# russellgeum/Digging-into-Self-Supervised-Monocular-Depth-Estimation

Measured on AMD Instinct MI355X. Metric: images/sec training, KITTI 192x640 batch 12/GPU, higher is better.
Workload: dtype f32; 1 GPU; configs[1]: kitti_eigen_zhou-shaped 192x640, batch 12/GPU, ResNet18 depth + separate ResNet18 pose, frame_ids [0,-1,1], 4 scales, automask, Adam, fp32; global_batch=12, parallelism=dp1

## Files before the change

### digging-into-self-supervised-monocular-depth-estimation_amd/csrc/norm_nhwc.hip

```cpp
#include "nhwc_common.hpp"

namespace mdx {
namespace nhwc {

constexpr int STATS_FWD_BLOCKS = 256;
constexpr int STATS_BWD_BLOCKS_F32 = 256, STATS_BWD_BLOCKS_BF16 = 384;
constexpr int STATS_MAX_BLOCKS = 384;
constexpr int APPLY_MAX_BLOCKS = 4096;
constexpr int STATS_ITERS = 8, APPLY_ITERS = 4;
static inline int stats_bwd_blocks(int dtype) { return dtype == MDX_F32 ? STATS_BWD_BLOCKS_F32 : STATS_BWD_BLOCKS_BF16; }

template <typename T>
__global__ __launch_bounds__(NB) void bn_nhwc_fwd_stats_kernel(const T *__restrict__ x, int M, int C, int CVB, int PL, int RB,
                                                               float *__restrict__ part)
{
    constexpr int N = VecN<T>::N;
    __shared__ float lds[2 * NB * N];
    const Pos p = position<N>(M, C, CVB, PL, RB);
    float a[N], q[N];
#pragma unroll
    for (int j = 0; j < N; ++j) a[j] = q[j] = 0.f;
    if (p.active) {
        const T *px = x + (size_t)p.g * M * C + (size_t)p.cv * N;
        auto acc = [&](const Vec<T, N> &v) {
// ... 241 lines not shown
    auto apply = [&](const Vec<T, N> &vd, const Vec<T, N> &vd2, const Vec<T, N> &vy, const Vec<T, N> &vx, size_t off) {
        Vec<T, N> wx, wr;
#pragma unroll
        for (int j = 0; j < N; ++j) {
            float d = to_float(vd.v[j]);
            if (pd2) d += to_float(vd2.v[j]);
            const float yv = !MASKX ? to_float(vy.v[j]) : to_float(from_float<T>(__builtin_fmaf(to_float(vx.v[j]), k0[j], shift[j])));
            const float dz = (relu && !(yv > 0.f)) ? 0.f : d;
            const float xh = (to_float(vx.v[j]) - mean[j]) * invstd[j];
            wx.v[j] = from_float<T>(k0[j] * (dz - mdz[j] - xh * mdzx[j]));
            wr.v[j] = from_float<T>(dz);
        }
        store_vec<T, N>(ox + off, wx);
        if (orr) store_vec<T, N>(orr + off, wr);
    };
    int r = p.r0 + p.pl;
    for (; r + PL < p.r1; r += 2 * PL) {
        const size_t o0 = (size_t)r * C, o1 = (size_t)(r + PL) * C;
        const Vec<T, N> d0 = load_vec<T, N>(pd + o0), d1 = load_vec<T, N>(pd + o1);
        Vec<T, N> y0 = {}, y1 = {};
        if (!MASKX) { y0 = load_vec<T, N>(py + o0); y1 = load_vec<T, N>(py + o1); }
        const Vec<T, N> x0 = load_vec<T, N>(px + o0), x1 = load_vec<T, N>(px + o1);
        Vec<T, N> e0 = {}, e1 = {};
        if (pd2) { e0 = load_vec<T, N>(pd2 + o0); e1 = load_vec<T, N>(pd2 + o1); }
        apply(d0, e0, y0, x0, o0);
        apply(d1, e1, y1, x1, o1);
    }
    for (; r < p.r1; r += PL) {
        const size_t o = (size_t)r * C;
        Vec<T, N> e = {}, yv = {};
        if (pd2) e = load_vec<T, N>(pd2 + o);
        if (!MASKX) yv = load_vec<T, N>(py + o);
        apply(load_vec<T, N>(pd + o), e, yv, load_vec<T, N>(px + o), o);
    }
}

}
}

using namespace mdx;
using namespace mdx::nhwc;

MDX_EXPORT size_t mdx_bn_nhwc_workspace_bytes(int B, int C, int H, int W, int groups, int dtype)
{
    if (B <= 0 || C <= 0 || H <= 0 || W <= 0 || groups <= 0 || !dtype_ok(dtype)) return 0;
    const Rows g = make_rows((long long)B * H * W, C, vec_elems(dtype), STATS_MAX_BLOCKS, STATS_ITERS);
    return ((size_t)groups * g.nblk * 2 * C + (size_t)groups * 2 * C) * sizeof(float);
}

static int nhwc_args_ok(int B, int C, int H, int W, int groups, int dtype)
{
    if (groups <= 0 || groups > 65535) return MDX_ERR_BAD_SHAPE;
    return nhwc_map_ok(B, C, H, W, dtype);
}

MDX_EXPORT int mdx_bn_act_nhwc_fwd(const void *x, const void *res, const float *gamma, const float *beta, float *run_mean,
                                   float *run_var, void *y, float *save_mean, float *save_invstd, int B, int C, int H, int W,
                                   int groups, float eps, float momentum, int relu, int dtype, void *workspace,
                                   size_t workspace_bytes, void *stream)
{
    if (!x || !gamma || !beta || !y || !save_mean || !save_invstd || !workspace) return MDX_ERR_NULL_POINTER;
    if ((run_mean == nullptr) != (run_var == nullptr)) return MDX_ERR_NULL_POINTER;
    const int bad = nhwc_args_ok(B, C, H, W, groups, dtype);
    if (bad) return bad;
    if (!aligned(x, 16) || !aligned(y, 16) || (res && !aligned(res, 16))) return MDX_ERR_MISALIGNED;
    if (workspace_bytes < mdx_bn_nhwc_workspace_bytes(B, C, H, W, groups, dtype)) return MDX_ERR_WORKSPACE;
    const int M = B * H * W, N = vec_elems(dtype);
    const Rows gs = make_rows(M, C, N, STATS_FWD_BLOCKS, STATS_ITERS), ga = make_rows(M, C, N, APPLY_MAX_BLOCKS, APPLY_ITERS);
    float *part = (float *)workspace;
    hipStream_t st = (hipStream_t)stream;
    const dim3 grid_s(gs.nblk, gs.t.ny, groups), grid_a(ga.nblk, ga.t.ny, groups), block(NB);
    dispatch_dtype(dtype, [&](auto t) {
        using T = typename decltype(t)::type;
        hipLaunchKernelGGL((bn_nhwc_fwd_stats_kernel<T>), grid_s, block, 0, st, (const T *)x, M, C, gs.t.CVB, gs.t.PL, gs.RB, part);
    });
    hipLaunchKernelGGL(bn_nhwc_fwd_finalize_kernel, dim3((C + FC - 1) / FC), dim3(FC * FS), 0, st, part, gs.nblk, C, groups, (double)M,
                       eps, momentum, save_mean, save_invstd, run_mean, run_var);
    dispatch_dtype(dtype, [&](auto t) {
        using T = typename decltype(t)::type;
        hipLaunchKernelGGL((bn_nhwc_fwd_apply_kernel<T>), grid_a, block, 0, st, (const T *)x, (const T *)res, gamma, beta, save_mean,
                           save_invstd, M, C, ga.t.CVB, ga.t.PL, ga.RB, relu, (T *)y);
    });
    return check_launch();
}

MDX_EXPORT int mdx_bn_act_nhwc_bwd(const void *dy, const void *dy2, const void *y, const void *x, const float *gamma,
                                   const float *beta, const float *save_mean, const float *save_invstd, void *dx, void *dres, float *dgamma,
                                   float *dbeta, int B, int C, int H, int W, int groups, int relu, int dtype, void *workspace,
                                   size_t workspace_bytes, void *stream)
{
    if (!dy || !x || !gamma || !save_mean || !save_invstd || !dx || !dgamma || !dbeta || !workspace)
        return MDX_ERR_NULL_POINTER;
    if (!y && (!relu || !beta || dres)) return MDX_ERR_NULL_POINTER;
    const int bad = nhwc_args_ok(B, C, H, W, groups, dtype);
    if (bad) return bad;
    if (!aligned(dy, 16) || (y && !aligned(y, 16)) || !aligned(x, 16) || !aligned(dx, 16) || (dy2 && !aligned(dy2, 16)) ||
        (dres && !aligned(dres, 16)))
        return MDX_ERR_MISALIGNED;
    if (workspace_bytes < mdx_bn_nhwc_workspace_bytes(B, C, H, W, groups, dtype)) return MDX_ERR_WORKSPACE;
    const int M = B * H * W, N = vec_elems(dtype);
    const Rows gs = make_rows(M, C, N, stats_bwd_blocks(dtype), STATS_ITERS), ga = make_rows(M, C, N, APPLY_MAX_BLOCKS, APPLY_ITERS);
    float *part = (float *)workspace;
    float *totals = part + (size_t)groups * gs.nblk * 2 * C;
    hipStream_t st = (hipStream_t)stream;
    const dim3 grid_s(gs.nblk, gs.t.ny, groups), grid_a(ga.nblk, ga.t.ny, groups), block(NB);
    const bool maskx = !y;
    dispatch_dtype_flag(dtype, maskx, [&](auto t, auto mx) {
        using T = typename decltype(t)::type;
        hipLaunchKernelGGL((bn_nhwc_bwd_stats_kernel<T, decltype(mx)::value>), grid_s, block, 0, st, (const T *)dy, (const T *)dy2,
                           (const T *)y, (const T *)x, gamma, beta, save_mean, save_invstd, M, C, gs.t.CVB, gs.t.PL, gs.RB, relu, part);
    });
    hipLaunchKernelGGL(bn_nhwc_bwd_finalize_kernel, dim3((C + FC - 1) / FC), dim3(FC * FS), 0, st, part, gs.nblk, C, groups, (double)M, totals,
                       dgamma, dbeta);
    dispatch_dtype_flag(dtype, maskx, [&](auto t, auto mx) {
        using T = typename decltype(t)::type;
        hipLaunchKernelGGL((bn_nhwc_bwd_apply_kernel<T, decltype(mx)::value>), grid_a, block, 0, st, (const T *)dy, (const T *)dy2,
                           (const T *)y, (const T *)x, gamma, beta, save_mean, save_invstd, totals, M, C, ga.t.CVB, ga.t.PL, ga.RB, relu,
                           (T *)dx, (T *)dres);
    });
    return check_launch();
}
```

### digging-into-self-supervised-monocular-depth-estimation_amd/mdx/functional.py

```python
import ctypes as C

import torch

from . import _lib
from ._lib import api, ptr, stream, workspace


def _f32c(t, keep_format=False):
    if t is not None and t.dtype != torch.float32:
        t = t.float()
    if t is None or t.is_contiguous() or (keep_format and t.is_contiguous(memory_format=torch.channels_last)):
        return t
    return t.contiguous()


def _byref(struct):
    return C.byref(struct) if struct is not None else None


class _ComposeProjection(torch.autograd.Function):
    @staticmethod
    def forward(ctx, K, T):
        K, T = _f32c(K), _f32c(T)
        B = K.shape[0]
        P = torch.empty(B, 3, 4, device=K.device, dtype=torch.float32)
        api.mdx_compose_projection(ptr(K), ptr(T), B, ptr(P), stream())
        ctx.save_for_backward(K, T)
        return P

    @staticmethod
    def backward(ctx, gP):
        K, T = ctx.saved_tensors
        gK = gT = None
# ... 918 lines not shown
        nws = api.mdx_bn_nhwc_workspace_bytes(Bg, Cc, H, W, groups, code) if cl else api.mdx_bn_workspace_bytes(Bg, Cc, H, W)
        ws = workspace(nws, x.device)
        fn = api.mdx_bn_act_nhwc_fwd if cl else api.mdx_bn_act_fwd
        fn(ptr(x, x.dtype, cl=cl), ptr(res, x.dtype, optional=True, cl=cl), ptr(weight), ptr(bias),
           ptr(running_mean, optional=True), ptr(running_var, optional=True), ptr(y, x.dtype, cl=cl), ptr(save_mean),
           ptr(save_invstd), Bg, Cc, H, W, groups, eps, momentum, int(relu), code, ptr(ws, torch.uint8), nws, stream())
        mask_from_x = cl and bool(relu) and res is None and x.dtype == torch.float32
        ctx.save_for_backward(x, bias if mask_from_x else y, weight, save_mean, save_invstd)
        ctx.meta = (bool(relu), res is not None, groups, cl, mask_from_x)
        ctx.mark_non_differentiable(*[t for t in (running_mean, running_var) if t is not None])
        ctx.set_materialize_grads(False)
        return (y, y.view_as(y)) if fork else y

    @staticmethod
    def backward(ctx, dy, dy2=None):
        x, y, weight, save_mean, save_invstd = ctx.saved_tensors
        relu, has_res, groups, cl, mask_from_x = ctx.meta
        bias = None
        if mask_from_x:
            y, bias = None, y
        dy, dy2 = _two_grads(dy, dy2, x.dtype, cl, fused_add=cl)
        if dy is None:
            return (None,) * 11
        B, Cc, H, W = x.shape
        Bg = B // groups
        code = _DTYPE_CODE[x.dtype]
        dx = torch.empty_like(x)
        dres = torch.empty_like(x) if has_res else None
        dgamma = torch.empty(Cc, device=x.device, dtype=torch.float32)
        dbeta = torch.empty(Cc, device=x.device, dtype=torch.float32)
        nws = api.mdx_bn_nhwc_workspace_bytes(Bg, Cc, H, W, groups, code) if cl else api.mdx_bn_workspace_bytes(Bg, Cc, H, W)
        ws = workspace(nws, x.device)
        if cl:
            api.mdx_bn_act_nhwc_bwd(
                ptr(dy, x.dtype, cl=True), ptr(dy2, x.dtype, optional=True, cl=True), ptr(y, x.dtype, optional=True, cl=True),
                ptr(x, x.dtype, cl=True), ptr(weight), ptr(bias, optional=True), ptr(save_mean), ptr(save_invstd),
                ptr(dx, x.dtype, cl=True), ptr(dres, x.dtype, optional=True, cl=True), ptr(dgamma), ptr(dbeta), Bg, Cc, H, W,
                groups, int(relu), code, ptr(ws, torch.uint8), nws, stream())
        else:
            api.mdx_bn_act_bwd(
                ptr(dy, x.dtype), ptr(y, x.dtype), ptr(x, x.dtype), ptr(weight), ptr(save_mean), ptr(save_invstd),
                ptr(dx, x.dtype), ptr(dres, x.dtype, optional=True), ptr(dgamma), ptr(dbeta), Bg, Cc, H, W, groups,
                int(relu), code, ptr(ws, torch.uint8), nws, stream())
        return (dx, dres, dgamma, dbeta) + (None,) * 7


def bn_act(x, weight, bias, running_mean, running_var, eps=1e-5, momentum=0.1, residual=None, relu=True, groups=1,
           fork=False):
    return _BnAct.apply(x, residual, weight, bias, running_mean, running_var, float(eps), float(momentum), bool(relu),
                        int(groups), bool(fork))


def bn_act_infer(x, weight, bias, running_mean, running_var, eps=1e-5, residual=None, relu=True, fork=False):
    B, Cc, H, W = x.shape
    code, cl, _ = _layout(x, "bn_act_infer", Cc)
    x, residual = _as(x, cl), _as(_residual("bn_act_infer", residual, x), cl)
    y = torch.empty_like(x)
    fn = api.mdx_bn_act_nhwc_infer if cl else api.mdx_bn_act_infer
    fn(ptr(x, x.dtype, cl=cl), ptr(residual, x.dtype, optional=True, cl=cl), ptr(_f32c(weight)),
       ptr(_f32c(bias)), ptr(_f32c(running_mean)), ptr(_f32c(running_var)), ptr(y, x.dtype, cl=cl), B, Cc, H, W, float(eps),
       int(bool(relu)), code, stream())
    return (y, y.view_as(y)) if fork else y


class _Param2Matrix(torch.autograd.Function):
    @staticmethod
    def forward(ctx, axisangle, translation, invert):
        aa, tr = _f32c(axisangle).reshape(-1, 3), _f32c(translation).reshape(-1, 3)
        N = aa.shape[0]
        if tr.shape[0] != N:
            raise _lib.MdxError("param2matrix: %d rotations, %d translations" % (N, tr.shape[0]))
        M = torch.empty(N, 4, 4, device=aa.device, dtype=torch.float32)
        api.mdx_param2matrix_fwd(ptr(aa), ptr(tr), N, int(invert), ptr(M), stream())
        ctx.save_for_backward(aa, tr)
        ctx.meta = (bool(invert), axisangle.shape, translation.shape)
        return M

    @staticmethod
    def backward(ctx, gM):
        aa, tr = ctx.saved_tensors
        invert, sa, st = ctx.meta
        gM = _f32c(gM)
        gaa, gtr = torch.empty_like(aa), torch.empty_like(tr)
# ... 119 lines not shown
```

### digging-into-self-supervised-monocular-depth-estimation_amd/model_layer/depth_encoder.py

```python
import os
import warnings

import numpy as np
import torch
import torch.nn as nn
import torch.nn.functional as TF



class BatchNorm2d(nn.BatchNorm2d):

    fused_min_elements = 0
    fused_eval = True
    _batch_groups = 1

    @staticmethod
    def batch_groups(groups, network):
        import contextlib

        @contextlib.contextmanager
        def scope():
            mods = [m for m in network.modules() if isinstance(m, BatchNorm2d)]
            prev = [m.__dict__.get("_batch_groups") for m in mods]
            for m in mods:
# ... 3 lines not shown
            finally:
                for m, p in zip(mods, prev):
                    if p is None:
                        m.__dict__.pop("_batch_groups", None)
                    else:
                        m._batch_groups = p
        return scope()

    def __init__(self, *args, **kwargs):
        super().__init__(*args, **kwargs)
        self._pending_batches = 0

    def forward(self, x):
        if self.momentum is None or not self.track_running_stats:
            return super().forward(x)
        groups = self._batch_groups if self.training else 1
        if groups > 1:
            return torch.cat([self._norm(c) for c in x.chunk(groups)])
        return self._norm(x)

    def _norm(self, x):
        if self.training:
            self._pending_batches += 1
        return TF.batch_norm(x, self.running_mean, self.running_var, self.weight, self.bias, self.training,
                             self.momentum, self.eps)

    def act(self, x, residual=None, relu=True, fork=False):
        if not self.training and self._eval_fused(x, residual):
            from mdx import functional as F
            if residual is not None and residual.dtype != x.dtype:
                residual = residual.to(x.dtype)
            return F.bn_act_infer(x, self.weight, self.bias, self.running_mean, self.running_var, self.eps,
                                  residual=residual, relu=relu, fork=fork)
        fused = (self.training and x.is_cuda and self.track_running_stats and self.momentum is not None
                 and self.affine and x.dtype in (torch.float32, torch.bfloat16) and x.dim() == 4
                 and torch.is_grad_enabled() and x.shape[0] % self._batch_groups == 0
                 and x.shape[0] * x.shape[2] * x.shape[3] >= self.fused_min_elements
                 and (x.shape[0] // self._batch_groups) * ((x.shape[2] * x.shape[3] + 8191) // 8192) <= 65535)
        if not fused:
            out = self(x)
            if residual is not None:
                out = out + residual
            out = TF.relu(out) if relu else out
            return (out, out) if fork else out
        from mdx import functional as F
        self._pending_batches += self._batch_groups
        if residual is not None and residual.dtype != x.dtype:
            residual = residual.to(x.dtype)
        return F.bn_act(x, self.weight, self.bias, self.running_mean, self.running_var, self.eps, self.momentum,
                        residual=residual, relu=relu, groups=self._batch_groups, fork=fork)

    def _eval_fused(self, x, residual):
        if not (self.fused_eval and x.is_cuda and x.dtype in (torch.float32, torch.bfloat16) and x.dim() == 4
                and self.track_running_stats and self.affine and self.running_mean is not None):
            return False
        return not torch.is_grad_enabled() or not any(
            t is not None and t.requires_grad for t in (x, residual, self.weight, self.bias))

    def _flush_counter(self):
        if self._pending_batches and self.num_batches_tracked is not None:
            self.num_batches_tracked += self._pending_batches
        self._pending_batches = 0

    def _save_to_state_dict(self, destination, prefix, keep_vars):
        self._flush_counter()
        super()._save_to_state_dict(destination, prefix, keep_vars)

    def _load_from_state_dict(self, *args, **kwargs):
        self._pending_batches = 0
        super()._load_from_state_dict(*args, **kwargs)

def _pair(x):
    return x if isinstance(x, tuple) else (x, x)


class BasicBlock(nn.Module):
    expansion = 1
    fork_output = True

    def __init__(self, inplanes, planes, stride=1, downsample=None):
        super().__init__()
        self.conv1 = nn.Conv2d(inplanes, planes, 3, stride, 1, bias=False)
        self.bn1 = BatchNorm2d(planes)
# ... 62 lines not shown
        downsample = None
        if stride != 1 or self.inplanes != planes * block.expansion:
            downsample = nn.Sequential(
                nn.Conv2d(self.inplanes, planes * block.expansion, 1, stride, bias=False),
                BatchNorm2d(planes * block.expansion))
        layers = [block(self.inplanes, planes, stride, downsample)]
        self.inplanes = planes * block.expansion
        layers += [block(self.inplanes, planes) for _ in range(1, blocks)]
        return nn.Sequential(*layers)


def _load_pretrained(model, num_layers, num_input_images):
    path = os.path.join(os.environ.get("MDX_RESNET_WEIGHTS", ""), "resnet%d.pth" % num_layers)
    if not os.path.isfile(path):
        warnings.warn("pretrained=True but %s not found (offline): using random init" % (path or "weights"))
        return
    loaded = torch.load(path, map_location="cpu")
    if num_input_images > 1:
        loaded["conv1.weight"] = torch.cat([loaded["conv1.weight"]] * num_input_images, 1) / num_input_images
    model.load_state_dict(loaded)


def resnet_multiimage_input(num_layers, pretrained=True, num_input_images=1):
    assert num_layers in [18, 50], "Can only run with 18 or 50 layer resnet"
    block, layers = _CFG[num_layers]
    model = ResNet(block, layers, num_input_images=num_input_images)
    if pretrained:
        _load_pretrained(model, num_layers, num_input_images)
    return model


class ResnetEncoder(nn.Module):

    def __init__(self, num_layers, pretrained, num_input_images=1):
        super().__init__()
        self.num_ch_enc = np.array([64, 64, 128, 256, 512])
        if num_layers not in _CFG:
            raise ValueError("{} is not a valid number of resnet layers".format(num_layers))
        if num_input_images > 1:
            self.encoder = resnet_multiimage_input(num_layers, pretrained, num_input_images)
        else:
            block, layers = _CFG[num_layers]
            self.encoder = ResNet(block, layers)
            if pretrained:
                _load_pretrained(self.encoder, num_layers, 1)
        if num_layers > 34:
            self.num_ch_enc[1:] *= 4

    fused_input = True

    def _normalised_input(self, input_image):
        from mdx import functional as F
        from mdx.layout import weight_layout
        stack = input_image if isinstance(input_image, F.FrameStack) else None
        if stack is None and torch.is_tensor(input_image) and input_image.dim() == 4 and input_image.shape[1] == 3:
            stack = F.FrameStack([[input_image]])
        if (self.fused_input and stack is not None and stack.ok() and weight_layout(self.encoder.conv1)
                and stack.blocks[0][0].numel() * len(stack.blocks) * len(stack.blocks[0]) < (1 << 31)):
            dt = torch.get_autocast_gpu_dtype() if torch.is_autocast_enabled() else torch.float32
            if dt in (torch.float32, torch.bfloat16):
                return F.encoder_input(stack, 0.45, 0.225, dt)
        if isinstance(input_image, F.FrameStack):
            input_image = input_image.tensor()
        return (input_image - 0.45) / 0.225

    def forward(self, input_image):
        from mdx.layout import to_layout, weight_layout
        self.features = []
        x = self._normalised_input(input_image)
        stem, stem_b = _pair(self.encoder.bn1.act(self.encoder.conv1(x), fork=BasicBlock.fork_output))
        self.features.append(stem)
        if (stem.is_cuda and stem.dtype in (torch.float32, torch.bfloat16)
                and stem.shape[0] * stem.shape[1] <= 65535):
            from mdx import functional as F
            x = F.maxpool3s2(stem_b, fork=BasicBlock.fork_output)
        else:
            x = self.encoder.maxpool(stem_b)
        for layer in (self.encoder.layer1, self.encoder.layer2, self.encoder.layer3, self.encoder.layer4):
            x = _pair(layer(to_layout(x, weight_layout(layer)) if x[0].is_cuda else x))
            self.features.append(x[0])
        return self.features
```

### digging-into-self-supervised-monocular-depth-estimation_amd/model_tool/loader.py

```python
import os

import torch
from torch.utils.data import DataLoader
from torch.utils.data.distributed import DistributedSampler

from model_layer import *
from model_loss import *
from .synthetic import SyntheticKITTI


def _opt(opt, name, default):
    return getattr(opt, name, default)


def collate_step_keys(samples):
    from torch.utils.data import default_collate
    from .processor import step_reads
    return default_collate([{k: v for k, v in s.items() if step_reads(k)} for s in samples])


def collate_raw_step_keys(samples):
    from model_loader.kitti import collate_raw
    from .processor import step_reads
    return collate_raw(samples, step_reads)
# ... 37 lines not shown
                                     is_training=is_training, geometry=_opt(opt, "synthetic_geometry", False))
        else:
            from model_loader import KITTIMonoDataset_v2, KITTIMonoStereoDataset
            from model_utility import readlines
            names = readlines(os.path.join(opt.splits, opt.datatype, "{}_files.txt".format(split)))
            cls = KITTIMonoDataset_v2 if opt.dataset == "kitti_mono" else KITTIMonoStereoDataset
            dataset = cls(opt.datapath, names, is_training, opt.frame_ids, opt.height, opt.width, ".jpg", len(opt.scales))
            dataset.uint8 = _opt(opt, "uint8_loader", False)
            dataset.gpu_prep = gpu_image_prep(opt, self.device)
            dataset.gpu_velo = dataset.gpu_prep and bool(int(_opt(opt, "gpu_velodyne", 0) or 0))
        sampler = None
        if self.distributed:
            sampler = DistributedSampler(dataset, self.world_size, self.rank, shuffle=shuffle, drop_last=True)
            shuffle = False
        workers = opt.num_workers
        if workers < 0:
            share = max(2, len(os.sched_getaffinity(0)) // max(1, min(self.world_size, torch.cuda.device_count() or 1)))
            workers = max(2, min(24, share + share // 2) if str(_opt(opt, "amp", "none")) == "bf16" else min(16, share))
        return DataLoader(dataset, opt.batch, shuffle, sampler=sampler, num_workers=workers,
                          drop_last=True, pin_memory=str(self.device).startswith("cuda"),
                          collate_fn=(collate_raw_step_keys if getattr(dataset, "gpu_prep", False) or getattr(dataset, "raw", False)
                                      else collate_step_keys if _opt(opt, "collate_step_keys", False) else None),
                          persistent_workers=workers > 0, prefetch_factor=(_opt(opt, "prefetch_factor", 4) if workers > 0 else None))

    def set_model(self):
        opt = self.opt
        self.model["encoder"] = ResnetEncoder(num_layers=opt.num_layers, pretrained=opt.weight_init)
        self.model["decoder"] = DepthDecoder(num_ch_enc=self.model["encoder"].num_ch_enc, scales=opt.scales)
        if opt.pose_type == "posecnn":
            self.model["pose_decoder"] = PoseCNN(num_input_frames=self.num_pose_frames)
        elif opt.pose_type == "shared":
            self.model["pose_decoder"] = PoseDecoder(self.model["encoder"].num_ch_enc, self.num_pose_frames)
        elif opt.pose_type == "separate":
            self.model["pose_encoder"] = ResnetEncoder(opt.num_layers, opt.weight_init, self.num_pose_frames)
            self.model["pose_decoder"] = PoseDecoder(self.model["pose_encoder"].num_ch_enc, num_input_features=1,
                                                     num_frames_to_predict_for=2)
        self.inv_projection = {0: Depth2PointCloud(opt.batch, opt.height, opt.width).to(self.device)}
        self.for_projection = {0: PointCloud2Pixel(opt.batch, opt.height, opt.width).to(self.device)}
        for key in self.model:
            self.model[key] = self.model[key].to(self.device)
        from mdx.layout import apply_plan
        plan = _opt(opt, "channels_last", "auto")
        if plan == "auto" and not str(self.device).startswith("cuda"):
            plan = "none"
        self.channels_last_stages = apply_plan(self.model, plan)
        for key in self.model:
            m = self.model[key]
            for name, p in m.named_parameters():
                if name.startswith("encoder.fc."):
                    p.requires_grad_(False)
            self.model[key] = m
            self.parameters += [p for p in m.parameters() if p.requires_grad]
        self.raw_model = self.model
        if self.distributed:
            from .parallel import grad_sync, broadcast_state, dp_graph_allowed
            broadcast_state(self.model.values())
            comm = {"fp32": None, "bf16": torch.bfloat16}[str(_opt(opt, "grad_comm", "fp32"))]
            captured = bool(_opt(opt, "graph", False)) and str(self.device).startswith("cuda") \
                and str(_opt(opt, "noise", "device")) != "cpu" and torch.distributed.get_backend() == "nccl"
            mb = int(_opt(opt, "bucket_mb", 0)) or ((1 << 20) if captured else 32)
            self.sync = grad_sync(self.parameters, bucket_mb=mb, comm_dtype=comm)

    def set_loss(self):
        self.loss["reprojection"] = ReprojectionLoss().to(self.device)
        self.loss["edge_aware"] = SmoothLoss().to(self.device)

    def set_optim(self):
# ... 44 lines not shown
```

### include/mdx.h

```cpp
#ifndef MDX_H
#define MDX_H

#include <stddef.h>
#include <stdint.h>

#ifdef __cplusplus
extern "C" {
#endif

#define MDX_VERSION 510
#define MDX_MAX_SRC 4
#define MDX_MAX_SCALES 4

typedef enum mdx_status {
    MDX_OK = 0,
    MDX_ERR_BAD_SHAPE = -1,
    MDX_ERR_NULL_POINTER = -2,
    MDX_ERR_WORKSPACE = -3,
    MDX_ERR_LAUNCH = -4,
    MDX_ERR_UNSUPPORTED = -5,
    MDX_ERR_MISALIGNED = -6
} mdx_status;

#define MDX_FLAG_AUTOMASK 1u
// ... 240 lines not shown
size_t mdx_decoder_glue_workspace_bytes(int B, int C1, int h, int w);
int mdx_decoder_glue_bwd(const void *gout, const void *raw, const float *bias, void *graw, void *gskip, float *dbias,
                         int B, int C1, int C2, int h, int w, int upsample, int elu, int in_dtype, int out_dtype,
                         void *workspace, size_t workspace_bytes, void *stream);

int mdx_maxpool3s2_fwd(const void *in, void *out, uint8_t *arg, int BC, int H, int W, int dtype, void *stream);
int mdx_maxpool3s2_bwd(const void *gout, const uint8_t *arg, void *gin, int BC, int H, int W, int dtype, void *stream);

size_t mdx_bn_workspace_bytes(int B, int C, int H, int W);
int mdx_bn_act_fwd(const void *x, const void *res, const float *gamma, const float *beta, float *run_mean,
                   float *run_var, void *y, float *save_mean, float *save_invstd, int B, int C, int H, int W,
                   int groups, float eps, float momentum, int relu, int dtype, void *workspace, size_t workspace_bytes,
                   void *stream);
int mdx_bn_act_bwd(const void *dy, const void *y, const void *x, const float *gamma, const float *save_mean,
                   const float *save_invstd, void *dx, void *dres, float *dgamma, float *dbeta, int B, int C, int H,
                   int W, int groups, int relu, int dtype, void *workspace, size_t workspace_bytes, void *stream);

int mdx_bn_act_infer(const void *x, const void *res, const float *gamma, const float *beta, const float *run_mean,
                     const float *run_var, void *y, int B, int C, int H, int W, float eps, int relu, int dtype,
                     void *stream);
int mdx_bn_act_nhwc_infer(const void *x, const void *res, const float *gamma, const float *beta, const float *run_mean,
                          const float *run_var, void *y, int B, int C, int H, int W, float eps, int relu, int dtype,
                          void *stream);

size_t mdx_bn_nhwc_workspace_bytes(int B, int C, int H, int W, int groups, int dtype);
int mdx_bn_act_nhwc_fwd(const void *x, const void *res, const float *gamma, const float *beta, float *run_mean,
                        float *run_var, void *y, float *save_mean, float *save_invstd, int B, int C, int H, int W,
                        int groups, float eps, float momentum, int relu, int dtype, void *workspace,
                        size_t workspace_bytes, void *stream);
int mdx_bn_act_nhwc_bwd(const void *dy, const void *dy2, const void *y, const void *x, const float *gamma,
                        const float *beta, const float *save_mean, const float *save_invstd, void *dx, void *dres, float *dgamma,
                        float *dbeta, int B, int C, int H, int W, int groups, int relu, int dtype, void *workspace,
                        size_t workspace_bytes, void *stream);
size_t mdx_bias_act_nhwc_workspace_bytes(int B, int C, int H, int W, int dtype);
int mdx_bias_act_nhwc_fwd(const void *x, const float *bias, void *y, int B, int C, int H, int W, int relu, int dtype, void *stream);
int mdx_bias_act_nhwc_bwd(const void *dy, const void *y, void *dx, float *dbias, int B, int C, int H, int W, int relu, int dtype,
                          void *workspace, size_t workspace_bytes, void *stream);
int mdx_mean_bias_nhwc_fwd(const void *x, const float *bias, float *out, int B, int C, int H, int W, float scale, int dtype,
                           void *stream);
int mdx_mean_bias_nhwc_bwd(const float *gout, void *dx, float *dbias, int B, int C, int H, int W, float scale, int dtype,
                           void *stream);

int mdx_encoder_input_nhwc(const float *const *src, int blocks, int groups, int n, int H, int W, float mean, float inv_std,
                           void *out, int dtype, void *stream);

size_t mdx_thin_conv3x3_wgrad_workspace_bytes(int B, int Cin, int Cout, int h, int w);
int mdx_thin_conv3x3_wgrad(const float *x, const float *gy, float *gweight, int64_t s_o, int64_t s_c, int64_t s_y, int64_t s_x, int B,
                           int Cin, int Cout, int h, int w, void *workspace, size_t workspace_bytes, void *stream);

size_t mdx_disp_head_nhwc_workspace_bytes(int B, int C, int h, int w, int dtype);
int mdx_disp_head_nhwc_fwd(const void *x, const float *weight, int64_t w_stride_c, int64_t w_stride_ky, int64_t w_stride_kx,
                           const float *bias, float *disp, int B, int C, int h, int w, int dtype, void *stream);
int mdx_disp_head_nhwc_bwd(const void *x, const float *weight, int64_t w_stride_c, int64_t w_stride_ky, int64_t w_stride_kx,
                           const float *gdisp, const float *disp, void *gx, float *gweight, float *gbias, int B, int C, int h,
                           int w, int dtype, void *workspace, size_t workspace_bytes, void *stream);
int mdx_decoder_glue_nhwc_fwd(const void *raw, const void *skip, const float *bias, void *out, int B, int C1, int C2,
                              int h, int w, int upsample, int elu, int in_dtype, int out_dtype, void *stream);
size_t mdx_decoder_glue_nhwc_workspace_bytes(int B, int C1, int h, int w, int in_dtype);
int mdx_decoder_glue_nhwc_bwd(const void *gout, const void *raw, const float *bias, void *graw, void *gskip,
                              float *dbias, int B, int C1, int C2, int h, int w, int upsample, int elu, int in_dtype,
                              int out_dtype, void *workspace, size_t workspace_bytes, void *stream);
int mdx_maxpool3s2_nhwc_fwd(const void *in, void *out, uint8_t *arg, int B, int C, int H, int W, int dtype,
                            void *stream);
int mdx_maxpool3s2_nhwc_bwd(const void *gout, const void *gout2, const uint8_t *arg, void *gin, int B, int C, int H,
                            int W, int dtype, void *stream);

// ... 69 lines not shown
```

Measured before the change: 826.7 images/s.

## Fuse stem BN+ReLU with maxpool and compute BN backward dz once

Adds a fused BN-apply+ReLU+3x3/s2 maxpool forward kernel for the encoder stem. It writes the pooled map and a uint8 argmax, and for the pose encoder it skips writing the full-resolution activation, since that stem feature is unused. It also adds a BN backward path for residual blocks that computes the masked gradient dz once in the stats kernel and stores it into dres. The apply kernel then reads dz instead of re-reading dy, dy2 and y. The aim is to cut memory traffic and kernel launches, at the cost of extra kernels and an env toggle, and the stem pool path reads nine overlapping taps per output.

```diff
diff --git a/digging-into-self-supervised-monocular-depth-estimation_amd/csrc/norm_nhwc.hip b/digging-into-self-supervised-monocular-depth-estimation_amd/csrc/norm_nhwc.hip
--- a/digging-into-self-supervised-monocular-depth-estimation_amd/csrc/norm_nhwc.hip
+++ b/digging-into-self-supervised-monocular-depth-estimation_amd/csrc/norm_nhwc.hip
@@ -297,6 +297,204 @@
         if (pd2) e = load_vec<T, N>(pd2 + o);
         if (!MASKX) yv = load_vec<T, N>(py + o);
         apply(load_vec<T, N>(pd + o), e, yv, load_vec<T, N>(px + o), o);
+    }
+}
+
+template <typename T>
+__global__ __launch_bounds__(NB) void bn_nhwc_bwd_stats_dz_kernel(const T *__restrict__ dy, const T *__restrict__ dy2,
+                                                                  const T *__restrict__ y, const T *__restrict__ x,
+                                                                  const float *__restrict__ save_mean,
+                                                                  const float *__restrict__ save_invstd, int M, int C, int CVB,
+                                                                  int PL, int RB, int relu, float *__restrict__ part,
+                                                                  T *__restrict__ dres)
+{
+    constexpr int N = VecN<T>::N;
+    __shared__ float lds[2 * NB * N];
+    const Pos p = position<N>(M, C, CVB, PL, RB);
+    float a[N], q[N];
+#pragma unroll
+    for (int j = 0; j < N; ++j) a[j] = q[j] = 0.f;
+    if (p.active) {
+        float mean[N], invstd[N];
+#pragma unroll
+        for (int j = 0; j < N; ++j) {
+            mean[j] = save_mean[(size_t)p.g * C + p.cv * N + j];
+            invstd[j] = save_invstd[(size_t)p.g * C + p.cv * N + j];
+        }
+        const size_t base = (size_t)p.g * M * C + (size_t)p.cv * N;
+        const T *pd = dy + base, *pd2 = dy2 ? dy2 + base : nullptr, *py = y + base, *px = x + base;
+        T *orr = dres + base;
+        auto acc = [&](const Vec<T, N> &vd, const Vec<T, N> &vd2, const Vec<T, N> &vy, const Vec<T, N> &vx, size_t off) {
+            Vec<T, N> wr;
+#pragma unroll
+            for (int j = 0; j < N; ++j) {
+                float d = to_float(vd.v[j]);
+                if (pd2) d += to_float(vd2.v[j]);
+                const float dz = (relu && !(to_float(vy.v[j]) > 0.f)) ? 0.f : d;
+                a[j] += dz;
+                q[j] = __builtin_fmaf(dz, (to_float(vx.v[j]) - mean[j]) * invstd[j], q[j]);
+                wr.v[j] = from_float<T>(dz);
+            }
+            store_vec<T, N>(orr + off, wr);
+        };
+        int r = p.r0 + p.pl;
+        constexpr int U = 2;
+        for (; r + (U - 1) * PL < p.r1; r += U * PL) {
+            Vec<T, N> d[U], e[U], yy[U], xx[U];
+#pragma unroll
+            for (int u = 0; u < U; ++u) {
+                const size_t o = (size_t)(r + u * PL) * C;
+                d[u] = load_vec<T, N>(pd + o);
+                yy[u] = load_vec<T, N>(py + o);
+                xx[u] = load_vec<T, N>(px + o);
+                e[u] = Vec<T, N>{};
+                if (pd2) e[u] = load_vec<T, N>(pd2 + o);
+            }
+#pragma unroll
+            for (int u = 0; u < U; ++u) acc(d[u], e[u], yy[u], xx[u], (size_t)(r + u * PL) * C);
+        }
+        for (; r < p.r1; r += PL) {
+            const size_t o = (size_t)r * C;
+            Vec<T, N> e = {};
+            if (pd2) e = load_vec<T, N>(pd2 + o);
+            acc(load_vec<T, N>(pd + o), e, load_vec<T, N>(py + o), load_vec<T, N>(px + o), o);
+        }
+    }
+    block_partials<N>(a, q, lds, CVB, PL, C, part + ((size_t)p.g * gridDim.x + blockIdx.x) * 2 * C);
+}
+
+template <typename T>
+__global__ __launch_bounds__(NB) void bn_nhwc_bwd_apply_dz_kernel(const T *__restrict__ dz_map, const T *__restrict__ x,
+                                                                  const float *__restrict__ gamma,
+                                                                  const float *__restrict__ save_mean,
+                                                                  const float *__restrict__ save_invstd,
+                                                                  const float *__restrict__ totals, int M, int C, int CVB, int PL,
+                                                                  int RB, T *__restrict__ dx)
+{
+    constexpr int N = VecN<T>::N;
+    const Pos p = position<N>(M, C, CVB, PL, RB);
+    if (!p.active) return;
+    float mean[N], invstd[N], k0[N], mdz[N], mdzx[N];
+#pragma unroll
+    for (int j = 0; j < N; ++j) {
+        const int c = p.cv * N + j;
+        mean[j] = save_mean[(size_t)p.g * C + c];
+        invstd[j] = save_invstd[(size_t)p.g * C + c];
+        k0[j] = gamma[c] * invstd[j];
+        mdz[j] = totals[((size_t)p.g * 2 + 0) * C + c];
+        mdzx[j] = totals[((size_t)p.g * 2 + 1) * C + c];
+    }
+    const size_t base = (size_t)p.g * M * C + (size_t)p.cv * N;
+    const T *pz = dz_map + base, *px = x + base;
+    T *ox = dx + base;
+    auto apply = [&](const Vec<T, N> &vz, const Vec<T, N> &vx, size_t off) {
+        Vec<T, N> wx;
+#pragma unroll
+        for (int j = 0; j < N; ++j) {
+            const float dz = to_float(vz.v[j]);
+            const float xh = (to_float(vx.v[j]) - mean[j]) * invstd[j];
+            wx.v[j] = from_float<T>(k0[j] * (dz - mdz[j] - xh * mdzx[j]));
+        }
+        store_vec<T, N>(ox + off, wx);
+    };
+    int r = p.r0 + p.pl;
+    for (; r + 3 * PL < p.r1; r += 4 * PL) {
+        const size_t o0 = (size_t)r * C, o1 = (size_t)(r + PL) * C, o2 = (size_t)(r + 2 * PL) * C, o3 = (size_t)(r + 3 * PL) * C;
+        const Vec<T, N> z0 = load_vec<T, N>(pz + o0), z1 = load_vec<T, N>(pz + o1), z2 = load_vec<T, N>(pz + o2), z3 = load_vec<T, N>(pz + o3);
+        const Vec<T, N> x0 = load_vec<T, N>(px + o0), x1 = load_vec<T, N>(px + o1), x2 = load_vec<T, N>(px + o2), x3 = load_vec<T, N>(px + o3);
+        apply(z0, x0, o0); apply(z1, x1, o1); apply(z2, x2, o2); apply(z3, x3, o3);
+    }
+    for (; r < p.r1; r += PL) {
+        const size_t o = (size_t)r * C;
+        apply(load_vec<T, N>(pz + o), load_vec<T, N>(px + o), o);
+    }
+}
+
+struct Pix { int b, y, x; };
+__host__ __device__ __forceinline__ Pix pix_of(int r, int H, int W)
+{
+    Pix p;
+    p.b = r / (H * W);
+    const int rem = r - p.b * H * W;
+    p.y = rem / W;
+    p.x = rem - p.y * W;
+    return p;
+}
+__device__ __forceinline__ void pix_step(Pix &p, const Pix &s, int H, int W)
+{
+    p.x += s.x;
+    p.y += s.y;
+    p.b += s.b;
+    if (p.x >= W) { p.x -= W; ++p.y; }
+    if (p.y >= H) { p.y -= H; ++p.b; }
+}
+
+template <typename T>
+__global__ __launch_bounds__(NB) void bn_pool_nhwc_fwd_apply_kernel(const T *__restrict__ x, const float *__restrict__ gamma,
+                                                                    const float *__restrict__ beta,
+                                                                    const float *__restrict__ save_mean,
+                                                                    const float *__restrict__ save_invstd, int B, int Mo, int C, int H,
+                                                                    int W, int Ho, int Wo, int CVB, int PL, int RB, Pix step,
+                                                                    T *__restrict__ y, T *__restrict__ pooled,
+                                                                    uint8_t *__restrict__ arg)
+{
+    constexpr int N = VecN<T>::N;
+    const Pos p = position<N>(Mo, C, CVB, PL, RB);
+    if (!p.active) return;
+    float scale[N], shift[N];
+#pragma unroll
+    for (int j = 0; j < N; ++j) {
+        const int c = p.cv * N + j;
+        scale[j] = gamma[c] * save_invstd[(size_t)p.g * C + c];
+        shift[j] = beta[c] - save_mean[(size_t)p.g * C + c] * scale[j];
+    }
+    const size_t c0 = (size_t)p.cv * N;
+    int r = p.r0 + p.pl;
+    Pix po = pix_of(r, Ho, Wo);
+    for (; r < p.r1; r += PL, pix_step(po, step, Ho, Wo)) {
+        const size_t img = ((size_t)p.g * B + po.b) * H * W * C + c0;
+        Vec<T, N> tap[9];
+        bool ok[9];
+#pragma unroll
+        for (int k = 0; k < 9; ++k) {
+            const int yy = 2 * po.y - 1 + k / 3, xx = 2 * po.x - 1 + k % 3;
+            ok[k] = yy >= 0 && yy < H && xx >= 0 && xx < W;
+            tap[k] = load_vec<T, N>(x + img + ((size_t)(ok[k] ? yy : 0) * W + (ok[k] ? xx : 0)) * C);
+        }
+#pragma unroll
+        for (int k = 0; k < 9; ++k)
+#pragma unroll
+            for (int j = 0; j < N; ++j) {
+                const float f = __builtin_fmaf(to_float(tap[k].v[j]), scale[j], shift[j]);
+                tap[k].v[j] = from_float<T>(f < 0.f ? 0.f : f);
+            }
+        Vec<T, N> o;
+        Vec<uint8_t, N> a;
+#pragma unroll
+        for (int j = 0; j < N; ++j) {
+            float best = -INFINITY;
+            int bi = -1;
+#pragma unroll
+            for (int k = 0; k < 9; ++k) {
+                if (!ok[k]) continue;
+                const float v = to_float(tap[k].v[j]);
+                if (bi < 0) bi = k;
+                if (v > best || v != v) { best = v; bi = k; }
+            }
+            o.v[j] = from_float<T>(best);
+            a.v[j] = (uint8_t)bi;
+        }
+        const size_t off = ((size_t)p.g * Mo + r) * C + c0;
+        store_vec<T, N>(pooled + off, o);
+        store_vec<uint8_t, N>(arg + off, a);
+        if (y) {
+#pragma unroll
+            for (int k = 4; k < 9; ++k) {
+                if (k == 6 || !ok[k]) continue;
+                const int yy = 2 * po.y - 1 + k / 3, xx = 2 * po.x - 1 + k % 3;
+                store_vec<T, N>(y + img + ((size_t)yy * W + xx) * C, tap[k]);
+            }
+        }
     }
 }
 
@@ -349,6 +547,14 @@
     return check_launch();
 }
 
+static int g_dz_once = 1;
+MDX_EXPORT int mdx_bn_dz_once(int on)
+{
+    const int was = g_dz_once;
+    g_dz_once = on != 0;
+    return was;
+}
+
 MDX_EXPORT int mdx_bn_act_nhwc_bwd(const void *dy, const void *dy2, const void *y, const void *x, const float *gamma,
                                    const float *beta, const float *save_mean, const float *save_invstd, void *dx, void *dres, float *dgamma,
                                    float *dbeta, int B, int C, int H, int W, int groups, int relu, int dtype, void *workspace,
@@ -370,6 +576,16 @@
     hipStream_t st = (hipStream_t)stream;
     const dim3 grid_s(gs.nblk, gs.t.ny, groups), grid_a(ga.nblk, ga.t.ny, groups), block(NB);
     const bool maskx = !y;
+    if (dres && dtype == MDX_F32 && g_dz_once) {
+        using T = float;
+        hipLaunchKernelGGL((bn_nhwc_bwd_stats_dz_kernel<T>), grid_s, block, 0, st, (const T *)dy, (const T *)dy2, (const T *)y, (const T *)x,
+                           save_mean, save_invstd, M, C, gs.t.CVB, gs.t.PL, gs.RB, relu, part, (T *)dres);
+        hipLaunchKernelGGL(bn_nhwc_bwd_finalize_kernel, dim3((C + FC - 1) / FC), dim3(FC * FS), 0, st, part, gs.nblk, C, groups, (double)M,
+                           totals, dgamma, dbeta);
+        hipLaunchKernelGGL((bn_nhwc_bwd_apply_dz_kernel<T>), grid_a, block, 0, st, (const T *)dres, (const T *)x, gamma, save_mean,
+                           save_invstd, totals, M, C, ga.t.CVB, ga.t.PL, ga.RB, (T *)dx);
+        return check_launch();
+    }
     dispatch_dtype_flag(dtype, maskx, [&](auto t, auto mx) {
         using T = typename decltype(t)::type;
         hipLaunchKernelGGL((bn_nhwc_bwd_stats_kernel<T, decltype(mx)::value>), grid_s, block, 0, st, (const T *)dy, (const T *)dy2,
@@ -385,3 +601,35 @@
     });
     return check_launch();
 }
+
+static int bn_pool_args_ok(int B, int C, int H, int W, int groups, int dtype)
+{
+    const int bad = nhwc_args_ok(B, C, H, W, groups, dtype);
+    if (bad) return bad;
+    return dtype == MDX_F32 ? MDX_OK : MDX_ERR_BAD_SHAPE;
+}
+
+MDX_EXPORT int mdx_bn_pool_nhwc_fwd(const void *x, const float *gamma, const float *beta, float *run_mean, float *run_var, void *y,
+                                    void *pooled, uint8_t *arg, float *save_mean, float *save_invstd, int B, int C, int H, int W,
+                                    int groups, float eps, float momentum, int dtype, void *workspace, size_t workspace_bytes,
+                                    void *stream)
+{
+    if (!x || !gamma || !beta || !pooled || !arg || !save_mean || !save_invstd || !workspace) return MDX_ERR_NULL_POINTER;
+    if ((run_mean == nullptr) != (run_var == nullptr)) return MDX_ERR_NULL_POINTER;
+    const int bad = bn_pool_args_ok(B, C, H, W, groups, dtype);
+    if (bad) return bad;
+    if (!aligned(x, 16) || !aligned(pooled, 16) || !aligned(arg, 8) || (y && !aligned(y, 16))) return MDX_ERR_MISALIGNED;
+    if (workspace_bytes < mdx_bn_nhwc_workspace_bytes(B, C, H, W, groups, dtype)) return MDX_ERR_WORKSPACE;
+    using T = float;
+    const int M = B * H * W, N = vec_elems(dtype), Ho = (H - 1) / 2 + 1, Wo = (W - 1) / 2 + 1, Mo = B * Ho * Wo;
+    const Rows gs = make_rows(M, C, N, STATS_FWD_BLOCKS, STATS_ITERS), ga = make_rows(Mo, C, N, APPLY_MAX_BLOCKS, APPLY_ITERS);
+    float *part = (float *)workspace;
+    hipStream_t st = (hipStream_t)stream;
+    const dim3 grid_s(gs.nblk, gs.t.ny, groups), grid_a(ga.nblk, ga.t.ny, groups), block(NB);
+    hipLaunchKernelGGL((bn_nhwc_fwd_stats_kernel<T>), grid_s, block, 0, st, (const T *)x, M, C, gs.t.CVB, gs.t.PL, gs.RB, part);
+    hipLaunchKernelGGL(bn_nhwc_fwd_finalize_kernel, dim3((C + FC - 1) / FC), dim3(FC * FS), 0, st, part, gs.nblk, C, groups, (double)M,
+                       eps, momentum, save_mean, save_invstd, run_mean, run_var);
+    hipLaunchKernelGGL((bn_pool_nhwc_fwd_apply_kernel<T>), grid_a, block, 0, st, (const T *)x, gamma, beta, save_mean, save_invstd, B, Mo,
+                       C, H, W, Ho, Wo, ga.t.CVB, ga.t.PL, ga.RB, pix_of(ga.t.PL, Ho, Wo), (T *)y, (T *)pooled, arg);
+    return check_launch();
+}
diff --git a/digging-into-self-supervised-monocular-depth-estimation_amd/mdx/functional.py b/digging-into-self-supervised-monocular-depth-estimation_amd/mdx/functional.py
--- a/digging-into-self-supervised-monocular-depth-estimation_amd/mdx/functional.py
+++ b/digging-into-self-supervised-monocular-depth-estimation_amd/mdx/functional.py
@@ -1,4 +1,5 @@
 import ctypes as C
+import os
 
 import torch
 
@@ -983,6 +984,8 @@
         nws = api.mdx_bn_nhwc_workspace_bytes(Bg, Cc, H, W, groups, code) if cl else api.mdx_bn_workspace_bytes(Bg, Cc, H, W)
         ws = workspace(nws, x.device)
         if cl:
+            if has_res:
+                _dz_once_from_env()
             api.mdx_bn_act_nhwc_bwd(
                 ptr(dy, x.dtype, cl=True), ptr(dy2, x.dtype, optional=True, cl=True), ptr(y, x.dtype, optional=True, cl=True),
                 ptr(x, x.dtype, cl=True), ptr(weight), ptr(bias, optional=True), ptr(save_mean), ptr(save_invstd),
@@ -1000,6 +1003,85 @@
            fork=False):
     return _BnAct.apply(x, residual, weight, bias, running_mean, running_var, float(eps), float(momentum), bool(relu),
                         int(groups), bool(fork))
+
+
+_dz_once_set = False
+
+
+def bn_dz_once(on):
+    global _dz_once_set
+    _dz_once_set = True
+    return bool(api.mdx_bn_dz_once(int(bool(on))))
+
+
+def _dz_once_from_env():
+    if not _dz_once_set:
+        bn_dz_once(os.environ.get("MDX_BN_DZ_ONCE", "1") != "0")
+
+
+def bn_act_pool_ok(x):
+    return _cl_map(x, (torch.float32,)) and _nhwc_ok(x.dtype, x.shape[1])
+
+
+class _BnActPool(torch.autograd.Function):
+
+    @staticmethod
+    def forward(ctx, x, weight, bias, running_mean, running_var, eps, momentum, groups, need_map):
+        B, Cc, H, W = x.shape
+        if not bn_act_pool_ok(x):
+            raise _lib.MdxError("bn_act_pool takes a channels-last float32 GPU map with C %% 4 == 0, got %s %s on %s"
+                                % (tuple(x.shape), x.dtype, x.device))
+        if B % groups:
+            raise _lib.MdxError("bn_act_pool: batch %d is not divisible into %d groups" % (B, groups))
+        weight, bias = _f32c(weight), _f32c(bias)
+        Ho, Wo = (H - 1) // 2 + 1, (W - 1) // 2 + 1
+        y = torch.empty_like(x) if need_map else None
+        pooled = torch.empty(B, Cc, Ho, Wo, device=x.device, dtype=x.dtype, memory_format=_CL)
+        arg = torch.empty(B, Cc, Ho, Wo, device=x.device, dtype=torch.uint8, memory_format=_CL)
+        save_mean = torch.empty(groups, Cc, device=x.device, dtype=torch.float32)
+        save_invstd = torch.empty(groups, Cc, device=x.device, dtype=torch.float32)
+        Bg = B // groups
+        nws = api.mdx_bn_nhwc_workspace_bytes(Bg, Cc, H, W, groups, 0)
+        ws = workspace(nws, x.device)
+        api.mdx_bn_pool_nhwc_fwd(ptr(x, x.dtype, cl=True), ptr(weight), ptr(bias), ptr(running_mean, optional=True),
+                                 ptr(running_var, optional=True), ptr(y, x.dtype, optional=True, cl=True),
+                                 ptr(pooled, x.dtype, cl=True), ptr(arg, torch.uint8, cl=True), ptr(save_mean), ptr(save_invstd),
+                                 Bg, Cc, H, W, groups, eps, momentum, 0, ptr(ws, torch.uint8), nws, stream())
+        ctx.save_for_backward(x, bias, weight, save_mean, save_invstd, arg)
+        ctx.groups = groups
+        ctx.mark_non_differentiable(*[t for t in (running_mean, running_var) if t is not None])
+        ctx.set_materialize_grads(False)
+        return y, pooled, pooled.view_as(pooled)
+
+    @staticmethod
+    def backward(ctx, dy, gpool, gpool2):
+        x, bias, weight, save_mean, save_invstd, arg = ctx.saved_tensors
+        groups = ctx.groups
+        dy, _ = _two_grads(dy, None, x.dtype, True, fused_add=True)
+        gpool, gpool2 = _two_grads(gpool, gpool2, x.dtype, True, fused_add=True)
+        if dy is None and gpool is None:
+            return (None,) * 9
+        B, Cc, H, W = x.shape
+        Bg = B // groups
+        gin = None
+        if gpool is not None:
+            gin = torch.empty_like(x)
+            api.mdx_maxpool3s2_nhwc_bwd(ptr(gpool, x.dtype, cl=True), ptr(gpool2, x.dtype, optional=True, cl=True),
+                                        ptr(arg, torch.uint8, cl=True), ptr(gin, x.dtype, cl=True), B, Cc, H, W, 0, stream())
+        dy, dy2 = _two_grads(dy, gin, x.dtype, True, fused_add=True)
+        dx = torch.empty_like(x)
+        dgamma = torch.empty(Cc, device=x.device, dtype=torch.float32)
+        dbeta = torch.empty(Cc, device=x.device, dtype=torch.float32)
+        nws = api.mdx_bn_nhwc_workspace_bytes(Bg, Cc, H, W, groups, 0)
+        ws = workspace(nws, x.device)
+        api.mdx_bn_act_nhwc_bwd(ptr(dy, x.dtype, cl=True), ptr(dy2, x.dtype, optional=True, cl=True), None, ptr(x, x.dtype, cl=True),
+                                ptr(weight), ptr(bias), ptr(save_mean), ptr(save_invstd), ptr(dx, x.dtype, cl=True), None,
+                                ptr(dgamma), ptr(dbeta), Bg, Cc, H, W, groups, 1, 0, ptr(ws, torch.uint8), nws, stream())
+        return (dx, dgamma, dbeta) + (None,) * 6
+
+
+def bn_act_pool(x, weight, bias, running_mean, running_var, eps=1e-5, momentum=0.1, groups=1, need_map=True):
+    return _BnActPool.apply(x, weight, bias, running_mean, running_var, float(eps), float(momentum), int(groups), bool(need_map))
 
 
 def bn_act_infer(x, weight, bias, running_mean, running_var, eps=1e-5, residual=None, relu=True, fork=False):
diff --git a/digging-into-self-supervised-monocular-depth-estimation_amd/model_layer/depth_encoder.py b/digging-into-self-supervised-monocular-depth-estimation_amd/model_layer/depth_encoder.py
--- a/digging-into-self-supervised-monocular-depth-estimation_amd/model_layer/depth_encoder.py
+++ b/digging-into-self-supervised-monocular-depth-estimation_amd/model_layer/depth_encoder.py
@@ -59,12 +59,7 @@
                 residual = residual.to(x.dtype)
             return F.bn_act_infer(x, self.weight, self.bias, self.running_mean, self.running_var, self.eps,
                                   residual=residual, relu=relu, fork=fork)
-        fused = (self.training and x.is_cuda and self.track_running_stats and self.momentum is not None
-                 and self.affine and x.dtype in (torch.float32, torch.bfloat16) and x.dim() == 4
-                 and torch.is_grad_enabled() and x.shape[0] % self._batch_groups == 0
-                 and x.shape[0] * x.shape[2] * x.shape[3] >= self.fused_min_elements
-                 and (x.shape[0] // self._batch_groups) * ((x.shape[2] * x.shape[3] + 8191) // 8192) <= 65535)
-        if not fused:
+        if not self._train_fused(x):
             out = self(x)
             if residual is not None:
                 out = out + residual
@@ -76,6 +71,27 @@
             residual = residual.to(x.dtype)
         return F.bn_act(x, self.weight, self.bias, self.running_mean, self.running_var, self.eps, self.momentum,
                         residual=residual, relu=relu, groups=self._batch_groups, fork=fork)
+
+    def _train_fused(self, x):
+        return (self.training and x.is_cuda and self.track_running_stats and self.momentum is not None
+                and self.affine and x.dtype in (torch.float32, torch.bfloat16) and x.dim() == 4
+                and torch.is_grad_enabled() and x.shape[0] % self._batch_groups == 0
+                and x.shape[0] * x.shape[2] * x.shape[3] >= self.fused_min_elements
+                and (x.shape[0] // self._batch_groups) * ((x.shape[2] * x.shape[3] + 8191) // 8192) <= 65535)
+
+    def act_pool(self, x, need_map=True, fork=False, fused=True, pool=None):
+        from mdx import functional as F
+        if (fused and self._train_fused(x) and F.bn_act_pool_ok(x)
+                and x.shape[0] * x.shape[1] <= 65535):
+            self._pending_batches += self._batch_groups
+            y, p1, p2 = F.bn_act_pool(x, self.weight, self.bias, self.running_mean, self.running_var, self.eps, self.momentum,
+                                      groups=self._batch_groups, need_map=need_map)
+            return y, ((p1, p2) if fork else p1)
+        y, y_b = _pair(self.act(x, fork=fork))
+        if (y.is_cuda and y.dtype in (torch.float32, torch.bfloat16)
+                and y.shape[0] * y.shape[1] <= 65535):
+            return y, F.maxpool3s2(y_b, fork=fork)
+        return y, (pool(y_b) if pool is not None else TF.max_pool2d(y_b, 3, 2, 1))
 
     def _eval_fused(self, x, residual):
         if not (self.fused_eval and x.is_cuda and x.dtype in (torch.float32, torch.bfloat16) and x.dim() == 4
@@ -204,8 +220,9 @@
 
 class ResnetEncoder(nn.Module):
 
-    def __init__(self, num_layers, pretrained, num_input_images=1):
-        super().__init__()
+    def __init__(self, num_layers, pretrained, num_input_images=1, stem_feature=True):
+        super().__init__()
+        self.stem_feature = bool(stem_feature)
         self.num_ch_enc = np.array([64, 64, 128, 256, 512])
         if num_layers not in _CFG:
             raise ValueError("{} is not a valid number of resnet layers".format(num_layers))
@@ -219,6 +236,7 @@
         if num_layers > 34:
             self.num_ch_enc[1:] *= 4
 
+    fused_stem = True
     fused_input = True
 
     def _normalised_input(self, input_image):
@@ -240,14 +258,9 @@
         from mdx.layout import to_layout, weight_layout
         self.features = []
         x = self._normalised_input(input_image)
-        stem, stem_b = _pair(self.encoder.bn1.act(self.encoder.conv1(x), fork=BasicBlock.fork_output))
-        self.features.append(stem)
-        if (stem.is_cuda and stem.dtype in (torch.float32, torch.bfloat16)
-                and stem.shape[0] * stem.shape[1] <= 65535):
-            from mdx import functional as F
-            x = F.maxpool3s2(stem_b, fork=BasicBlock.fork_output)
-        else:
-            x = self.encoder.maxpool(stem_b)
+        stem, x = self.encoder.bn1.act_pool(self.encoder.conv1(x), need_map=self.stem_feature, fork=BasicBlock.fork_output,
+                                            fused=self.fused_stem, pool=self.encoder.maxpool)
+        self.features.append(stem if self.stem_feature else None)
         for layer in (self.encoder.layer1, self.encoder.layer2, self.encoder.layer3, self.encoder.layer4):
             x = _pair(layer(to_layout(x, weight_layout(layer)) if x[0].is_cuda else x))
             self.features.append(x[0])
diff --git a/digging-into-self-supervised-monocular-depth-estimation_amd/model_tool/loader.py b/digging-into-self-supervised-monocular-depth-estimation_amd/model_tool/loader.py
--- a/digging-into-self-supervised-monocular-depth-estimation_amd/model_tool/loader.py
+++ b/digging-into-self-supervised-monocular-depth-estimation_amd/model_tool/loader.py
@@ -93,7 +93,7 @@
         elif opt.pose_type == "shared":
             self.model["pose_decoder"] = PoseDecoder(self.model["encoder"].num_ch_enc, self.num_pose_frames)
         elif opt.pose_type == "separate":
-            self.model["pose_encoder"] = ResnetEncoder(opt.num_layers, opt.weight_init, self.num_pose_frames)
+            self.model["pose_encoder"] = ResnetEncoder(opt.num_layers, opt.weight_init, self.num_pose_frames, stem_feature=False)
             self.model["pose_decoder"] = PoseDecoder(self.model["pose_encoder"].num_ch_enc, num_input_features=1,
                                                      num_frames_to_predict_for=2)
         self.inv_projection = {0: Depth2PointCloud(opt.batch, opt.height, opt.width).to(self.device)}
diff --git a/include/mdx.h b/include/mdx.h
--- a/include/mdx.h
+++ b/include/mdx.h
@@ -296,6 +296,11 @@
                         const float *beta, const float *save_mean, const float *save_invstd, void *dx, void *dres, float *dgamma,
                         float *dbeta, int B, int C, int H, int W, int groups, int relu, int dtype, void *workspace,
                         size_t workspace_bytes, void *stream);
+int mdx_bn_dz_once(int on);
+int mdx_bn_pool_nhwc_fwd(const void *x, const float *gamma, const float *beta, float *run_mean, float *run_var, void *y,
+                         void *pooled, uint8_t *arg, float *save_mean, float *save_invstd, int B, int C, int H, int W,
+                         int groups, float eps, float momentum, int dtype, void *workspace, size_t workspace_bytes,
+                         void *stream);
 size_t mdx_bias_act_nhwc_workspace_bytes(int B, int C, int H, int W, int dtype);
 int mdx_bias_act_nhwc_fwd(const void *x, const float *bias, void *y, int B, int C, int H, int W, int relu, int dtype, void *stream);
 int mdx_bias_act_nhwc_bwd(const void *dy, const void *y, void *dx, float *dbias, int B, int C, int H, int W, int relu, int dtype,
```

Measured after the change: 836.3 images/s, median of 6. 1.01x the previous value.
